# migoox/genome-downsampler

Measured on AMD Instinct MI355X. Metric: Mreads/s selected at target coverage M=100, higher is better.
Workload: dtype u32

## Files before the change

### genome-downsampler_amd/csrc/kernels/pass_major.inc.hip

```cpp
static constexpr int kPmPass = 8192;
__host__ __device__ inline uint32_t pm_stride_of(uint32_t n_ranges) { return (uint32_t)kPmPass + 64u * n_ranges; }
static constexpr int kPmThreads = 512;
static constexpr int kPmWaves = kPmThreads / 64;
static constexpr int kPmPassesPerWg = 4;
static constexpr size_t kPmSortLds = ((size_t)kPmPass + kPmWaves * 256 + 2 * 256 + 16 + 2 * kPmPassesPerWg * 256 + kPmWaves * 3 * 128) * sizeof(uint32_t);
static constexpr uint32_t kPmExcPerWave = 128;

static constexpr uint32_t kPmFlatDigits = 32;
static constexpr uint32_t kPmStageWords = 10240;
static constexpr uint32_t kPmFlatSlots = 8;
static_assert(kPmStageWords >= (uint32_t)kPmPass + kPmFlatDigits * 63u, "a padded pass of 32 slices fits the stage");
static_assert(kPmStageWords <= (uint32_t)kPmPass + kPmWaves * 3u * kPmExcPerWave, "the stage's tail aliases s_exc and nothing else");
static_assert(kPmFlatDigits == 1u << kPmLaneFormBits, "a pass the lane counts rank is a pass the flat write-out takes");

#ifndef QMCP_PM_MIN_WAVES
#define QMCP_PM_MIN_WAVES 4
#endif
__global__ __launch_bounds__(kPmThreads, QMCP_PM_MIN_WAVES) void k_pm_prepare_sort(
    const uint32_t* __restrict__ starts, const uint32_t* __restrict__ ends, uint32_t n,
    const uint64_t* __restrict__ contig_read_off, const uint64_t* __restrict__ contig_pos_off, uint32_t n_contigs,
    const uint32_t* __restrict__ vbase ,
    uint32_t shift, uint32_t stride ,
    uint16_t* __restrict__ keys16, uint16_t* __restrict__ idx16,
    uint32_t* __restrict__ cnt_tab, uint32_t* __restrict__ lst_tab, uint32_t pitch ,
// ... 298 lines not shown
        for (int x = 1; x < kPmWaves; ++x) { mn = min(mn, s_red[0][x]); mx = max(mx, s_red[1][x]); bad |= s_red[2][x]; }
        if (mn < __hip_atomic_load(&stats[0], __ATOMIC_RELAXED, __HIP_MEMORY_SCOPE_AGENT)) atomicMin(&stats[0], mn);
        if (mx > __hip_atomic_load(&stats[1], __ATOMIC_RELAXED, __HIP_MEMORY_SCOPE_AGENT)) atomicMax(&stats[1], mx);
        if (bad) atomicOr(&stats[2], 1u);
    }
}

static constexpr uint32_t kPmDescrY = 8;
static constexpr uint32_t kPmWorkWords = 256u * kPmDescrY * 2u;

struct PmSlot { uint32_t slot0, nv, pass; };
template <bool kVector>
__device__ __forceinline__ PmSlot pm_unpack(uint32_t dsc, bool has, uint32_t stride) {
    PmSlot s;
    s.pass = dsc >> 15;
    s.slot0 = has ? (kVector ? __umul24(s.pass, stride) : s.pass * stride) + (((dsc >> 6) & 511u) << 6) : 0u;
    s.nv = has ? (dsc & 63u) + 1u : 0u;
    return s;
}

__device__ __forceinline__ void pm_row_part(uint32_t pitch, uint32_t& P_beg, uint32_t& P_end) {
    const uint32_t per = (pitch + kPmDescrY - 1u) / kPmDescrY;
    P_beg = min(pitch, blockIdx.y * per);
    P_end = min(pitch, (blockIdx.y + 1u) * per);
}

__global__ __launch_bounds__(256) void k_pm_row_sums(const uint32_t* __restrict__ cnt_tab, const uint32_t* __restrict__ lstw,
                                                     uint32_t pitch, uint32_t* __restrict__ work) {
    __shared__ uint32_t s_red[2][4];
    const uint32_t d = blockIdx.x;
    uint32_t P_beg, P_end;
    pm_row_part(pitch, P_beg, P_end);
    uint32_t pad = 0, tru = 0;
    for (uint32_t P0 = P_beg + threadIdx.x; P0 < P_end; P0 += 4u * 256u) {
        uint32_t c[4], w[4];
#pragma unroll
        for (int u = 0; u < 4; ++u) {
            const uint32_t P = min(P0 + (uint32_t)u * 256u, P_end - 1u);
            c[u] = cnt_tab[(size_t)d * pitch + P];
            w[u] = lstw[(size_t)d * pitch + P];
        }
#pragma unroll
        for (int u = 0; u < 4; ++u)
            if (P0 + (uint32_t)u * 256u < P_end) { pad += c[u]; tru += w[u] >> 16; }
    }
    pad = wave_sum_u32(pad);
    tru = wave_sum_u32(tru);
    if ((threadIdx.x & 63u) == 0u) { s_red[0][threadIdx.x >> 6] = pad; s_red[1][threadIdx.x >> 6] = tru; }
    __syncthreads();
    if (threadIdx.x == 0) {
        uint32_t* const out = work + ((size_t)d * kPmDescrY + blockIdx.y) * 2u;
        out[0] = s_red[0][0] + s_red[0][1] + s_red[0][2] + s_red[0][3];
        out[1] = s_red[1][0] + s_red[1][1] + s_red[1][2] + s_red[1][3];
    }
}

__global__ __launch_bounds__(256) void k_pm_tables(uint32_t* tab, const uint32_t* __restrict__ lstw, uint32_t pitch,
                                                   uint32_t n_groups ,
                                                   uint32_t* __restrict__ desc, const uint32_t* __restrict__ work,
                                                   uint32_t* __restrict__ range_start,
                                                   uint32_t* __restrict__ max_load ,
                                                   uint32_t* __restrict__ clear16 ) {
    __shared__ uint32_t s_red[4], s_red2[4], s_base, s_tile[2][4][4];
    const uint32_t d = blockIdx.x, y = blockIdx.y, tid = threadIdx.x;
    const uint32_t lane = tid & 63u, wv = tid >> 6;
    const bool first = d == 0u && y == 0u;
    uint32_t rp = 0, rt = 0, before = 0;
    {
        const uint4* const src = reinterpret_cast<const uint4*>(work + (size_t)tid * kPmDescrY * 2u);
        uint4 q[kPmDescrY / 2u];
#pragma unroll
        for (uint32_t k = 0; k < kPmDescrY / 2u; ++k) q[k] = src[k];
#pragma unroll
        for (uint32_t k = 0; k < kPmDescrY / 2u; ++k) {
            if (2u * k < y) before += q[k].x;
            if (2u * k + 1u < y) before += q[k].z;
            rp += q[k].x + q[k].z;
            rt += q[k].y + q[k].w;
        }
    }
    {
        const uint32_t inc = wave_incl_scan_add(rp);
        if (lane == 63u) s_red[wv] = inc;
        __syncthreads();
        uint32_t base = 0;
        for (uint32_t x = 0; x < wv; ++x) base += s_red[x];
        if (tid == d) s_base = base + inc - rp + before;
        if (first && tid == 255u) tab[(size_t)256u * pitch] = base + inc;
        __syncthreads();
    }
    if (first) {
        if (clear16 != nullptr && tid < 16u) clear16[tid] = 0u;
        const uint32_t inc = wave_incl_scan_add(rt);
        const uint32_t mx = wave_max_u32(rt), mxp = wave_max_u32(rp);
        if (lane == 63u) s_red[wv] = inc;
        __syncthreads();
        uint32_t base = 0;
        for (uint32_t x = 0; x < wv; ++x) base += s_red[x];
        range_start[tid] = base + inc - rt;
        if (tid == 255u) range_start[256] = base + inc;
        __syncthreads();
        if (lane == 0u) { s_red[wv] = mx; s_red2[wv] = mxp; }
        __syncthreads();
        if (tid == 0) {
            max_load[0] = max(max(s_red[0], s_red[1]), max(s_red[2], s_red[3]));
            max_load[1] = max(max(s_red2[0], s_red2[1]), max(s_red2[2], s_red2[3])) >> 6;
        }
    }
    uint32_t P_beg, P_end;
    pm_row_part(pitch, P_beg, P_end);
    uint32_t carry = s_base;
    uint32_t round = 0;
    for (uint32_t P0 = P_beg; P0 < P_end; P0 += 4u * 256u, round ^= 1u) {
        uint32_t c[4], w[4], inc[4];
#pragma unroll
        for (int u = 0; u < 4; ++u) {
            const uint32_t P = P0 + (uint32_t)u * 256u + tid;
            const bool in = P < P_end;
            const size_t at = (size_t)d * pitch + min(P, P_end - 1u);
            c[u] = tab[at];
            w[u] = lstw[at];
            if (!in) { c[u] = 0u; w[u] = 0u; }
        }
#pragma unroll
        for (int u = 0; u < 4; ++u) {
            inc[u] = wave_incl_scan_add(c[u]);
            if (lane == 63u) s_tile[round][u][wv] = inc[u];
        }
        __syncthreads();
#pragma unroll
        for (int u = 0; u < 4; ++u) {
            uint32_t base = carry;
            for (uint32_t x = 0; x < wv; ++x) base += s_tile[round][u][x];
            carry += s_tile[round][u][0] + s_tile[round][u][1] + s_tile[round][u][2] + s_tile[round][u][3];
            const uint32_t P = P0 + (uint32_t)u * 256u + tid;
            if (P >= P_end) continue;
            const uint32_t t = base + inc[u] - c[u];
            tab[(size_t)d * pitch + P] = t;
            const uint32_t cnt = w[u] >> 16;
            if (cnt == 0u) continue;
            const uint32_t g = t >> 6;
            const uint32_t n_ws = (cnt + 63u) >> 6;
            for (uint32_t j = 0; j < n_ws; ++j)
                if (g + j < n_groups)
                    desc[g + j] = (P << 15) | (((w[u] & 0xFFFFu) + j) << 6) | (min(64u, cnt - 64u * j) - 1u);
        }
    }
}

__device__ __forceinline__ uint32_t pm_grid_pos0(const uint32_t* __restrict__ grid, uint32_t r) { return grid[r]; }
__device__ __forceinline__ uint32_t pm_grid_live(const uint32_t* __restrict__ grid, uint32_t r) { return grid[kPmGridRows + r]; }
__device__ __forceinline__ uint32_t pm_grid_contig(const uint32_t* __restrict__ grid, uint32_t r) { return grid[2u * kPmGridRows + r]; }

#ifndef QMCP_PM_OFFSETS_U
#define QMCP_PM_OFFSETS_U 8
#endif
__global__ __launch_bounds__(1024) void k_pm_offsets(const uint16_t* __restrict__ keys16, const uint32_t* __restrict__ desc,
                                                     const uint32_t* __restrict__ Tp, uint32_t pitch,
                                                     const uint32_t* __restrict__ range_start ,
                                                     const uint32_t* __restrict__ grid,
                                                     uint32_t shift, uint32_t stride, uint32_t ltot, uint32_t* __restrict__ boff,
                                                     uint32_t* __restrict__ empty_positions) {
    extern __shared__ uint32_t s_cnt32[];
#define PADDED(i) ((i) + ((i) >> 5))
    __shared__ uint32_t s_wsum[16], s_esum[16];
    const uint32_t range = blockIdx.x, width = 1u << shift;
    const uint32_t pos0 = pm_grid_pos0(grid, range), live = pm_grid_live(grid, range);
    const uint32_t lo_p = Tp[(size_t)range * pitch], hi_p = Tp[(size_t)(range + 1) * pitch];
    const uint32_t g0 = lo_p >> 6, n_ws = (hi_p - lo_p) >> 6;
    const uint32_t lo = range_start[range];
    for (uint32_t i = threadIdx.x; i < width; i += blockDim.x) s_cnt32[PADDED(i)] = 0;
    __syncthreads();
    const uint32_t lane = threadIdx.x & 63u, nw = blockDim.x >> 6;
    const uint32_t w = (uint32_t)__builtin_amdgcn_readfirstlane((int)(threadIdx.x >> 6));
    const uint32_t sub = lane >> 4, l16 = lane & 15u;
    constexpr int kU = QMCP_PM_OFFSETS_U;
    const uint32_t n_quads = (n_ws + 3u) >> 2;
    uint32_t dsc[kU];
    auto ask_descriptors = [&](uint32_t q0) {
#pragma unroll
        for (int u = 0; u < kU; ++u) dsc[u] = desc[g0 + min(4u * (q0 + (uint32_t)u * nw) + sub, n_ws - 1u)];
    };
    if (n_ws != 0u) ask_descriptors(w);
    for (uint32_t q0 = w; q0 < n_quads; q0 += kU * nw) {
        uint2 v[kU];
        uint32_t nv[kU];
#pragma unroll
        for (int u = 0; u < kU; ++u) {
            const PmSlot at = pm_unpack<true>(dsc[u], 4u * (q0 + (uint32_t)u * nw) + sub < n_ws, stride);
            nv[u] = at.nv;
            v[u] = *reinterpret_cast<const uint2*>(keys16 + at.slot0 + 4u * l16);
        }
        if (q0 + kU * nw < n_quads) ask_descriptors(q0 + kU * nw);
#pragma unroll
        for (int u = 0; u < kU; ++u) {
            const uint32_t e = 4u * l16;
            if (e < nv[u]) atomicAdd(&s_cnt32[PADDED(v[u].x & 0xFFFFu)], 1u);
            if (e + 1 < nv[u]) atomicAdd(&s_cnt32[PADDED(v[u].x >> 16)], 1u);
            if (e + 2 < nv[u]) atomicAdd(&s_cnt32[PADDED(v[u].y & 0xFFFFu)], 1u);
            if (e + 3 < nv[u]) atomicAdd(&s_cnt32[PADDED(v[u].y >> 16)], 1u);
        }
    }
    __syncthreads();
    const uint32_t per = width >= 1024u ? width >> 10 : 1u;
    const uint32_t firstp = threadIdx.x * per;
    uint32_t sum = 0, empties = 0;
    if (firstp < width)
        for (uint32_t qq = 0; qq < per; ++qq) {
            const uint32_t cq = s_cnt32[PADDED(firstp + qq)];
            sum += cq;
            empties += (cq == 0 && firstp + qq < live) ? 1u : 0u;
        }
    const uint32_t inc = wave_incl_scan_add(sum);
    const uint32_t wv = threadIdx.x >> 6;
    if (lane == 63) s_wsum[wv] = inc;
    if (empty_positions != nullptr) {
        empties = wave_sum_u32(empties);
        if (lane == 0) s_esum[wv] = empties;
    }
    __syncthreads();
    if (empty_positions != nullptr && threadIdx.x == 0) {
        uint32_t total = 0;
        for (uint32_t x = 0; x < nw; ++x) total += s_esum[x];
        if (total != 0) atomicAdd(empty_positions, total);
    }
    uint32_t run = lo + inc - sum;
    for (uint32_t x = 0; x < wv; ++x) run += s_wsum[x];
    if (firstp < width)
        for (uint32_t qq = 0; qq < per; ++qq) {
            const uint32_t cq = s_cnt32[PADDED(firstp + qq)];
            s_cnt32[PADDED(firstp + qq)] = run;
            run += cq;
        }
    __syncthreads();
    for (uint32_t i = threadIdx.x; i < live; i += blockDim.x) boff[pos0 + i] = s_cnt32[PADDED(i)];
    if (range == gridDim.x - 1u && threadIdx.x == 0) boff[ltot] = range_start[kPmGridRows];
#undef PADDED
}

struct EvQuota { const uint32_t* sev; const uint32_t* lastns; const uint64_t* poff; uint32_t n_contigs, ell; };

__device__ __forceinline__ uint32_t pm_settle_groups(const uint16_t* __restrict__ keys16, const uint16_t* __restrict__ idx16,
                                                     const uint32_t* __restrict__ desc, uint32_t g0, uint32_t n_ws,
                                                     uint32_t stride, const uint2* amb, uint32_t namb, uint32_t w,
                                                     uint32_t lane, unsigned long long* __restrict__ mask) {
    const uint64_t gt_mask = lane == 63 ? 0ull : ~((2ull << lane) - 1ull);
    uint32_t kept = 0;
    constexpr int kSteps = 16, kE = 2;
    constexpr uint32_t stride_k = 16;
    for (uint32_t k0 = w; k0 < namb; k0 += kE * stride_k) {
        uint32_t key[kE][kSteps], dscv[kE] , p[kE], skip[kE], c_of[kE];
#pragma unroll
        for (int x = 0; x < kE; ++x) {
            const uint32_t k = k0 + (uint32_t)x * stride_k;
            const uint2 ent = k < namb ? amb[k] : make_uint2(0u, 0u);
            c_of[x] = ent.x >> 15;
            p[x] = k < namb ? ent.x & 0x7FFFu : 0xFFFFFFFFu;
            skip[x] = ent.y;
            const uint32_t ws = 16u * c_of[x] + (lane & 15u);
            dscv[x] = ws < n_ws ? desc[g0 + ws] : 0u;
        }
#pragma unroll
        for (int x = 0; x < kE; ++x) {
#pragma unroll
            for (int t = 0; t < kSteps; ++t) {
                const uint32_t dsc = (uint32_t)__builtin_amdgcn_readlane((int)dscv[x], t);
                key[x][t] = keys16[pm_unpack<false>(dsc, 16u * c_of[x] + (uint32_t)t < n_ws, stride).slot0 + lane];
            }
        }
#pragma unroll
        for (int x = 0; x < kE; ++x) {
#pragma unroll
            for (int t = kSteps - 1; t >= 0; --t) {
                const uint32_t dsc = (uint32_t)__builtin_amdgcn_readlane((int)dscv[x], t);
                const PmSlot at = pm_unpack<false>(dsc, 16u * c_of[x] + (uint32_t)t < n_ws, stride);
                const bool member = lane < at.nv && key[x][t] == p[x];
                const uint64_t m = __ballot(member);
                if (m == 0) continue;
                const uint32_t above = (uint32_t)__popcll(m & gt_mask);
                if (member && above >= skip[x]) {
                    const uint32_t v = at.pass * (uint32_t)kPmPass + idx16[at.slot0 + lane];
                    atomicOr(&mask[v >> 6], 1ull << (v & 63u));
                }
                const uint32_t in_step = (uint32_t)__popcll(m);
                kept += in_step > skip[x] ? in_step - skip[x] : 0u;
                skip[x] = skip[x] > in_step ? skip[x] - in_step : 0u;
            }
        }
    }
    return kept;
}

__global__ __launch_bounds__(1024) void k_pm_walk(const uint16_t* __restrict__ keys16, const uint16_t* __restrict__ idx16,
                                                  const uint32_t* __restrict__ desc,
                                                  const uint32_t* __restrict__ Tp, uint32_t pitch,
                                                  const uint32_t* __restrict__ range_start ,
                                                  const uint32_t* __restrict__ grid,
                                                  uint32_t shift, uint32_t stride,
                                                  const uint32_t* __restrict__ boff, const uint32_t* __restrict__ selend,
                                                  EvQuota evq,
                                                  unsigned long long* __restrict__ mask,
                                                  uint2* __restrict__ amb_lists, int lists_by_records,
                                                  unsigned long long* __restrict__ kept_total) {
    extern __shared__ int32_t s_q[];
    __shared__ uint32_t s_namb, s_kept;
    __shared__ uint32_t s_ring[16][128];
    const uint32_t range = blockIdx.x, width = 1u << shift;
    const uint32_t pos0 = pm_grid_pos0(grid, range), live = pm_grid_live(grid, range);
    const uint32_t tid = threadIdx.x, nthreads = blockDim.x;
    const uint32_t lane = tid & 63u;
    const uint32_t w = (uint32_t)__builtin_amdgcn_readfirstlane((int)(tid >> 6));
    const uint32_t lo_p = Tp[(size_t)range * pitch];
    const uint32_t hi_p = Tp[(size_t)(range + 1) * pitch];
    if (lo_p >= hi_p) return;
    const uint32_t g0 = lo_p >> 6, n_ws = (hi_p - lo_p) >> 6;
    const uint32_t n_chunks = (n_ws + 15u) >> 4;
    const uint32_t lo_true = range_start[range];
    uint2* const amb = amb_lists + (lists_by_records ? (size_t)lo_true : (size_t)range * width);
    if (evq.sev != nullptr) {
        const uint32_t c_range = pm_grid_contig(grid, range);
        for (uint32_t i0 = tid; i0 < live; i0 += 8 * nthreads) {
            uint32_t src[8], back[8];
#pragma unroll
            for (int u = 0; u < 8; ++u) {
                const uint32_t p = pos0 + min(i0 + u * nthreads, live - 1);
                uint32_t c_lo = c_range, c_hi = c_range + 1u;
                if (c_range == kPmNoContig) { c_lo = 0; c_hi = evq.n_contigs; }
                while (c_hi - c_lo > 1) {
                    const uint32_t mid = (c_lo + c_hi) >> 1;
                    if ((uint32_t)evq.poff[mid] <= p) c_lo = mid; else c_hi = mid;
                }
                const uint32_t base = (uint32_t)evq.poff[c_lo];
                const uint32_t k = (p - base) / evq.ell;
                src[u] = p;
                back[u] = k - evq.lastns[(size_t)(base / (4u * evq.ell) + c_lo) * 4u + k];
            }
#pragma unroll
            for (int u = 0; u < 8; ++u) src[u] = evq.sev[src[u] - back[u] * evq.ell];
#pragma unroll
            for (int u = 0; u < 8; ++u)
                if (i0 + u * nthreads < live) s_q[i0 + u * nthreads] = (int32_t)src[u];
        }
    } else
    for (uint32_t i0 = tid; i0 < live; i0 += 8 * nthreads) {
        uint32_t a[8], b[8];
#pragma unroll
        for (int u = 0; u < 8; ++u) {
            const uint32_t i = min(i0 + u * nthreads, live - 1);
            a[u] = selend[pos0 + i];
            b[u] = boff[pos0 + i];
        }
#pragma unroll
        for (int u = 0; u < 8; ++u)
            if (i0 + u * nthreads < live) s_q[i0 + u * nthreads] = (int32_t)(a[u] - b[u]);
    }
    if (tid == 0) { s_namb = 0; s_kept = 0; }
    __syncthreads();

#define QMCP_PM_RING "v96", "v97", "v98", "v99", "v100", "v101", "v102", "v103", "v104", "v105", "v106", "v107", "v108", "v109", "v110", "v111", "v112", "v113", "v114", "v115", "v116", "v117", "v118", "v119"
#define QMCP_PM_KEYREG(k) "v" QMCP_PM_STR(QMCP_PM_CAT(QMCP_PM_KEY_, k))
#define QMCP_PM_DSCREG(k) "v" QMCP_PM_STR(QMCP_PM_CAT(QMCP_PM_DSC_, k))
#define QMCP_PM_IDXREG(k) "v" QMCP_PM_STR(QMCP_PM_CAT(QMCP_PM_IDX_, k))
#define QMCP_PM_STR(x) QMCP_PM_STR2(x)
#define QMCP_PM_STR2(x) #x
#define QMCP_PM_CAT(a, b) QMCP_PM_CAT2(a, b)
#define QMCP_PM_CAT2(a, b) a##b
#define QMCP_PM_KEY_0 96
#define QMCP_PM_KEY_1 97
#define QMCP_PM_KEY_2 98
#define QMCP_PM_KEY_3 99
#define QMCP_PM_KEY_4 100
#define QMCP_PM_KEY_5 101
#define QMCP_PM_KEY_6 102
#define QMCP_PM_KEY_7 103
#define QMCP_PM_DSC_0 104
#define QMCP_PM_DSC_1 105
#define QMCP_PM_DSC_2 106
#define QMCP_PM_DSC_3 107
#define QMCP_PM_DSC_4 108
#define QMCP_PM_DSC_5 109
#define QMCP_PM_DSC_6 110
#define QMCP_PM_DSC_7 111
#define QMCP_PM_IDX_0 112
#define QMCP_PM_IDX_1 113
#define QMCP_PM_IDX_2 114
#define QMCP_PM_IDX_3 115
#define QMCP_PM_IDX_4 116
#define QMCP_PM_IDX_5 117
#define QMCP_PM_IDX_6 118
#define QMCP_PM_IDX_7 119
    static_assert(kRankDepth == 8, "the ring registers are named for eight slots");
    struct Slot { uint32_t slot0, nv, read0; bool has; };
    auto desc_offset = [&](uint32_t c) -> uint32_t {
        return (g0 + min(16u * c + w, n_ws - 1u)) * 4u;
    };
    auto slot_of = [&](uint32_t dsc, uint32_t c) -> Slot {
        const bool has = 16u * c + w < n_ws;
        const PmSlot at = pm_unpack<true>(dsc, has, stride);
        Slot s;
        s.slot0 = at.slot0;
        s.nv = at.nv;
        s.read0 = at.pass * (uint32_t)kPmPass;
        s.has = has;
        return s;
    };
    uint32_t kept = 0;
    uint32_t cur = 0, flushed = 0;
    uint32_t* const ring = s_ring[w];
#define QMCP_PM_STEP(K, KF)                                                                                                   \
    {                                                                                                                         \
        const uint32_t c = c0 + (uint32_t)(K);                                                                                \
        uint32_t key, dsc, idx;                                                                                               \
        asm volatile("s_waitcnt vmcnt(19)\n\tv_mov_b32 %0, " QMCP_PM_KEYREG(K) "\n\tv_mov_b32 %1, " QMCP_PM_DSCREG(K)          \
                     "\n\tv_mov_b32 %2, " QMCP_PM_IDXREG(K)                                                                   \
                     : "=v"(key), "=v"(dsc), "=v"(idx) : : QMCP_PM_RING, "memory");                                                      \
        const Slot at = S[K];                                                                                                 \
        const bool valid = lane < at.nv;                                                                                      \
        int32_t old = 0;                                                                                                      \
        if (valid) old = atomicSub(&s_q[key], 1);                                         \
        S[KF] = slot_of(dsc, c + 7u);                                                                                         \
        asm volatile("global_load_ushort " QMCP_PM_KEYREG(KF) ", %0, %1\n\tglobal_load_ushort " QMCP_PM_IDXREG(KF) ", %0, %2"   \
                     "\n\tglobal_load_dword " QMCP_PM_DSCREG(K) ", %3, %4"                                                    \
                     : : "v"((S[KF].slot0 + lane) * 2u), "s"(keys16), "s"(idx16), "v"(desc_offset(c + 15u)), "s"(desc)        \
                     : QMCP_PM_RING, "memory");                                                                               \
        __syncthreads();                                                                                                      \
        int32_t aft = 0;                                                                                                      \
        if (valid) aft = s_q[key];                                                                                            \
        const bool keep = valid && old > 0 && aft >= 0;                                                                       \
        if (valid && old == 1 && aft < 0) {                                                                                   \
            const uint32_t k = atomicAdd(&s_namb, 1u);                                                                        \
            amb[k] = make_uint2((c << 15) | key, (uint32_t)(-aft));                                 \
        }                                                                                                                     \
        __syncthreads();                                               \
        if (at.has) {                                                    \
            const uint64_t kb = __ballot(keep);                                                                               \
            const uint32_t cw = (uint32_t)__popcll(kb);                                                                       \
            if (keep) ring[(cur + __builtin_amdgcn_mbcnt_hi((uint32_t)(kb >> 32), __builtin_amdgcn_mbcnt_lo((uint32_t)kb, 0u))) & 127u] = at.read0 + idx; \
            cur += cw;                                                                                                        \
            if (cur - flushed >= 64u) {                                                                          \
                const uint32_t v = ring[(flushed + lane) & 127u];                                                             \
                atomicOr(&mask[v >> 6], 1ull << (v & 63u));                                                                   \
                flushed += 64u;                                                                                               \
            }                                                                                                                 \
        }                                                                                                                     \
    }
    Slot S[kRankDepth];
    {
        uint32_t d0[kRankDepth - 1];
#pragma unroll
        for (int k = 0; k < kRankDepth - 1; ++k) d0[k] = desc[desc_offset((uint32_t)k) / 4u];
#pragma unroll
        for (int k = 0; k < kRankDepth - 1; ++k) S[k] = slot_of(d0[k], (uint32_t)k);
        S[kRankDepth - 1] = Slot{0u, 0u, 0u, false};
#define QMCP_PM_ASK_KEYS(K) asm volatile("global_load_ushort " QMCP_PM_KEYREG(K) ", %0, %1\n\tglobal_load_ushort " QMCP_PM_IDXREG(K) ", %0, %2" : : "v"((S[K].slot0 + lane) * 2u), "s"(keys16), "s"(idx16) : QMCP_PM_RING, "memory");
#define QMCP_PM_ASK_DSC(K) asm volatile("global_load_dword " QMCP_PM_DSCREG(K) ", %0, %1" : : "v"(desc_offset(7u + (uint32_t)(K))), "s"(desc) : QMCP_PM_RING, "memory");
        QMCP_PM_ASK_KEYS(0) QMCP_PM_ASK_KEYS(1) QMCP_PM_ASK_KEYS(2) QMCP_PM_ASK_KEYS(3) QMCP_PM_ASK_KEYS(4) QMCP_PM_ASK_KEYS(5) QMCP_PM_ASK_KEYS(6)
        QMCP_PM_ASK_DSC(0) QMCP_PM_ASK_DSC(1) QMCP_PM_ASK_DSC(2) QMCP_PM_ASK_DSC(3) QMCP_PM_ASK_DSC(4) QMCP_PM_ASK_DSC(5) QMCP_PM_ASK_DSC(6) QMCP_PM_ASK_DSC(7)
        asm volatile("s_waitcnt vmcnt(0)" : : : QMCP_PM_RING, "memory");
#undef QMCP_PM_ASK_KEYS
#undef QMCP_PM_ASK_DSC
    }
    for (uint32_t c0 = 0; c0 < n_chunks; c0 += kRankDepth) {
        QMCP_PM_STEP(0, 7) QMCP_PM_STEP(1, 0) QMCP_PM_STEP(2, 1) QMCP_PM_STEP(3, 2)
        QMCP_PM_STEP(4, 3) QMCP_PM_STEP(5, 4) QMCP_PM_STEP(6, 5) QMCP_PM_STEP(7, 6)
    }
#undef QMCP_PM_STEP
    asm volatile("s_waitcnt vmcnt(0)" : : : QMCP_PM_RING, "memory");
    if (lane < cur - flushed) {
        const uint32_t v = ring[(flushed + lane) & 127u];
        atomicOr(&mask[v >> 6], 1ull << (v & 63u));
    }
    kept = cur;
    __syncthreads();
    kept += pm_settle_groups(keys16, idx16, desc, g0, n_ws, stride, amb, s_namb, w, lane, mask);
    if (lane == 0 && kept) atomicAdd(&s_kept, kept);
    __syncthreads();
    if (tid == 0 && s_kept) atomicAdd(kept_total, (unsigned long long)s_kept);
}

uint32_t pm_pitch(uint32_t n) { return part_pass_pitch(n); }
uint32_t pm_pass() { return (uint32_t)kPmPass; }
uint32_t pm_stride(uint32_t n_ranges) { return pm_stride_of(n_ranges); }
size_t pm_slots(uint32_t n, uint32_t n_ranges) { return (size_t)pm_pitch(n) * pm_stride(n_ranges); }
uint32_t pm_work_words() { return kPmWorkWords; }
uint32_t pm_exc_slots(uint32_t n) { return pm_pitch(n) * kPmWaves * kPmExcPerWave + kNuOverflow; }
bool pm_rank_scratch_by_records(uint32_t shift, uint32_t n_ranges, uint32_t n) { return (size_t)n < ((size_t)n_ranges << shift); }
size_t pm_rank_scratch_bytes(uint32_t shift, uint32_t n_ranges, uint32_t n) {
    const size_t by_pos = (size_t)n_ranges << shift;
    return (by_pos < (size_t)n ? by_pos : (size_t)n) * sizeof(uint2) + 64;
}
void launch_pm_prepare_sort(hipStream_t st, const uint32_t* starts, const uint32_t* ends, uint32_t n,
                            const uint64_t* d_roff, const uint64_t* d_poff, uint32_t n_contigs, uint32_t shift,
                            uint32_t n_ranges, const uint32_t* d_grid,
                            uint16_t* keys16, uint16_t* idx16, uint32_t* cnt_tab, uint32_t* lst_tab,
                            uint32_t* stats, unsigned long long* zero_mask, uint32_t ell_reg, uint32_t* exc,
                            uint32_t exc_cap, uint32_t* exc_cnt) {
    const uint32_t pitch = pm_pitch(n);
    if (pitch == 0) return;
    (void)hipFuncSetAttribute((const void*)k_pm_prepare_sort, hipFuncAttributeMaxDynamicSharedMemorySize, (int)kPmSortLds);
    hipLaunchKernelGGL(k_pm_prepare_sort, dim3(pitch / kPmPassesPerWg), dim3(kPmThreads), kPmSortLds, st, starts, ends, n,
                       d_roff, d_poff, n_contigs, d_grid + 3u * kPmGridRows, shift, pm_stride(n_ranges), keys16, idx16,
                       cnt_tab, lst_tab, pitch, stats, zero_mask, exc != nullptr ? ell_reg : 0u, exc, exc_cap, exc_cnt);
    if (exc != nullptr && ell_reg != 0u)
        hipLaunchKernelGGL(k_nu_count_groups, dim3(32), dim3(256), 0, st, exc_cnt, pitch * kPmWaves, stats);
}
void launch_pm_row_sums(hipStream_t st, const uint32_t* cnt_tab, const uint32_t* lstw, uint32_t n, uint32_t* work) {
    const uint32_t pitch = pm_pitch(n);
    if (pitch == 0) return;
    hipLaunchKernelGGL(k_pm_row_sums, dim3(256, kPmDescrY), dim3(256), 0, st, cnt_tab, lstw, pitch, work);
}
void launch_pm_tables(hipStream_t st, uint32_t* tab, const uint32_t* lstw, uint32_t n, uint32_t n_ranges,
                      uint32_t* desc, const uint32_t* work, uint32_t* range_start, uint32_t* max_load, uint32_t* clear16) {
    const uint32_t pitch = pm_pitch(n);
    if (pitch == 0) return;
    const uint32_t s64 = pm_stride(n_ranges) / 64u;
    hipLaunchKernelGGL(k_pm_tables, dim3(256, kPmDescrY), dim3(256), 0, st, tab, lstw, pitch, pitch * s64, desc, work,
                       range_start, max_load, clear16);
}
void launch_pm_offsets(hipStream_t st, const uint16_t* keys16, const uint32_t* desc, const uint32_t* Tp, uint32_t n,
                       const uint32_t* range_start, uint32_t shift, uint32_t n_ranges, const uint32_t* d_grid, uint32_t ltot,
                       uint32_t* boff, uint32_t* empty_positions) {
    const size_t width = (size_t)1 << shift;
    const size_t lds = (width + width / 32 + 1) * sizeof(uint32_t);
    (void)hipFuncSetAttribute((const void*)k_pm_offsets, hipFuncAttributeMaxDynamicSharedMemorySize, (int)lds);
    hipLaunchKernelGGL(k_pm_offsets, dim3(n_ranges), dim3(1024), lds, st, keys16, desc, Tp, pm_pitch(n), range_start, d_grid,
                       shift, pm_stride(n_ranges), ltot, boff, empty_positions);
}
void launch_pm_walk(hipStream_t st, const uint16_t* keys16, const uint16_t* idx16, const uint32_t* desc, const uint32_t* Tp,
                    uint32_t n, const uint32_t* range_start, uint32_t shift, uint32_t n_ranges, const uint32_t* d_grid,
                    const uint32_t* boff, const uint32_t* selend, unsigned long long* mask, unsigned long long* kept_total, void* scratch,
                    bool scratch_by_records, const uint32_t* ev_sev, const uint32_t* ev_lastns,
                    const uint64_t* d_poff, uint32_t n_contigs, uint32_t ell) {
    const EvQuota evq{ev_sev, ev_lastns, d_poff, n_contigs, ell};
    const size_t lds = (((size_t)1 << shift) + 1) * sizeof(uint32_t);
    (void)hipFuncSetAttribute((const void*)k_pm_walk, hipFuncAttributeMaxDynamicSharedMemorySize, (int)lds);
    hipLaunchKernelGGL(k_pm_walk, dim3(n_ranges), dim3(1024), lds, st, keys16, idx16, desc, Tp, pm_pitch(n), range_start, d_grid, shift,
                       pm_stride(n_ranges), boff, selend, evq, mask, (uint2*)scratch, scratch_by_records ? 1 : 0,
                       kept_total);
}
```

### genome-downsampler_amd/csrc/qmcp_kernels.hip

```cpp
#include <hip/hip_runtime.h>
#include <stdint.h>

#include <type_traits>

#include "qmcp_kernels.h"
#include "target_table.h"

namespace qmcp {

static constexpr int kWave = 64;
static constexpr uint32_t kInf = 0x40000000u;

#include "kernels/wave_primitives.inc.hip"
#include "kernels/prepare_scan.inc.hip"
#include "kernels/radix_sort.inc.hip"
#include "kernels/ranked_route.inc.hip"
#include "kernels/bucket_offsets.inc.hip"
#include "kernels/sweep_uniform.inc.hip"
#include "kernels/sweep_segments.inc.hip"
#include "kernels/sweep_uniform_pipelines.inc.hip"
#include "kernels/sweep_uniform_events.inc.hip"
#include "kernels/sweep_mixed.inc.hip"
#include "kernels/mark_and_next_rows.inc.hip"
#include "kernels/launchers.inc.hip"
#include "kernels/pm_lane_rank.inc.hip"
#include "kernels/pass_major.inc.hip"
#include "kernels/near_uniform.inc.hip"
#include "kernels/by_contig.inc.hip"
#include "kernels/ladder.inc.hip"
#include "kernels/amplicon_by_contig.inc.hip"
#include "kernels/quality_cells.inc.hip"
#include "kernels/targets.inc.hip"
#include "kernels/depth_report.inc.hip"
#include "kernels/depth_track.inc.hip"
#include "kernels/stratified.inc.hip"
#include "kernels/dedup.inc.hip"
#include "kernels/start_cap.inc.hip"
#include "kernels/profile.inc.hip"
#include "kernels/pairs.inc.hip"
#include "kernels/templates.inc.hip"
#include "kernels/templates_profile.inc.hip"
#include "kernels/fragments.inc.hip"
#include "kernels/ceiling.inc.hip"
#include "kernels/proportional.inc.hip"
#include "kernels/budget.inc.hip"
#include "kernels/mean_depth.inc.hip"
#include "kernels/thresholds.inc.hip"
#include "kernels/replicates.inc.hip"

}
```

Before: 134,300.

## Pipeline pass-major offset counting, settling, and event quotas; add stamp probes

```diff
diff --git a/genome-downsampler_amd/csrc/kernels/pass_major.inc.hip b/genome-downsampler_amd/csrc/kernels/pass_major.inc.hip
--- a/genome-downsampler_amd/csrc/kernels/pass_major.inc.hip
+++ b/genome-downsampler_amd/csrc/kernels/pass_major.inc.hip
@@ -474,8 +474,44 @@
 __device__ __forceinline__ uint32_t pm_grid_live(const uint32_t* __restrict__ grid, uint32_t r) { return grid[kPmGridRows + r]; }
 __device__ __forceinline__ uint32_t pm_grid_contig(const uint32_t* __restrict__ grid, uint32_t r) { return grid[2u * kPmGridRows + r]; }
 
+#ifdef QMCP_PM_STAMP
+__device__ unsigned long long g_pm_stamps[2][kPmGridRows][8];
+__device__ __forceinline__ unsigned long long pm_stamp() {
+    unsigned long long t;
+    asm volatile("s_memtime %0\n\ts_waitcnt lgkmcnt(0)" : "=s"(t) : : "memory");
+    return t;
+}
+__device__ __forceinline__ unsigned long long pm_stamp_after(uint32_t dep) {
+    unsigned long long t;
+    asm volatile("s_memtime %0\n\ts_waitcnt lgkmcnt(0)" : "=s"(t) : "v"(dep) : "memory");
+    return t;
+}
+__device__ __forceinline__ unsigned long long pm_stamp_real() {
+    unsigned long long t;
+    asm volatile("s_memrealtime %0\n\ts_waitcnt lgkmcnt(0)" : "=s"(t) : : "memory");
+    return t;
+}
+#define QMCP_PM_STAMPS unsigned long long pm_t[5] = {0, 0, 0, 0, 0}; const unsigned long long pm_r0 = pm_stamp_real();
+#define QMCP_PM_STAMP_AT(i) pm_t[i] = pm_stamp();
+#define QMCP_PM_STAMP_AFTER(i, dep) pm_t[i] = pm_stamp_after(dep);
+#define QMCP_PM_STAMPS_OUT(kernel)                                                                         \
+    if (threadIdx.x == 0) {                                                                                \
+        unsigned long long* const row = g_pm_stamps[kernel][blockIdx.x];                                   \
+        for (int i = 0; i < 5; ++i) row[i] = pm_t[i];                                                      \
+        row[5] = 1ull; row[6] = pm_r0; row[7] = pm_stamp_real();                                           \
+    }
+#else
+#define QMCP_PM_STAMPS
+#define QMCP_PM_STAMP_AT(i)
+#define QMCP_PM_STAMP_AFTER(i, dep)
+#define QMCP_PM_STAMPS_OUT(kernel)
+#endif
+
+#ifndef QMCP_PM_OFFSETS_REC
+#define QMCP_PM_OFFSETS_REC 8
+#endif
 #ifndef QMCP_PM_OFFSETS_U
-#define QMCP_PM_OFFSETS_U 8
+#define QMCP_PM_OFFSETS_U 4
 #endif
 __global__ __launch_bounds__(1024) void k_pm_offsets(const uint16_t* __restrict__ keys16, const uint32_t* __restrict__ desc,
                                                      const uint32_t* __restrict__ Tp, uint32_t pitch,
@@ -483,47 +519,70 @@
                                                      const uint32_t* __restrict__ grid,
                                                      uint32_t shift, uint32_t stride, uint32_t ltot, uint32_t* __restrict__ boff,
                                                      uint32_t* __restrict__ empty_positions) {
-    extern __shared__ uint32_t s_cnt32[];
+    extern __shared__ __align__(16) uint32_t s_cnt32[];
 #define PADDED(i) ((i) + ((i) >> 5))
     __shared__ uint32_t s_wsum[16], s_esum[16];
     const uint32_t range = blockIdx.x, width = 1u << shift;
+    QMCP_PM_STAMPS
+    QMCP_PM_STAMP_AT(0)
     const uint32_t pos0 = pm_grid_pos0(grid, range), live = pm_grid_live(grid, range);
     const uint32_t lo_p = Tp[(size_t)range * pitch], hi_p = Tp[(size_t)(range + 1) * pitch];
     const uint32_t g0 = lo_p >> 6, n_ws = (hi_p - lo_p) >> 6;
     const uint32_t lo = range_start[range];
-    for (uint32_t i = threadIdx.x; i < width; i += blockDim.x) s_cnt32[PADDED(i)] = 0;
-    __syncthreads();
     const uint32_t lane = threadIdx.x & 63u, nw = blockDim.x >> 6;
     const uint32_t w = (uint32_t)__builtin_amdgcn_readfirstlane((int)(threadIdx.x >> 6));
-    const uint32_t sub = lane >> 4, l16 = lane & 15u;
     constexpr int kU = QMCP_PM_OFFSETS_U;
-    const uint32_t n_quads = (n_ws + 3u) >> 2;
+    constexpr uint32_t kRec = QMCP_PM_OFFSETS_REC;
+    static_assert(kRec == 4 || kRec == 8, "a lane loads 8 or 16 bytes");
+    const uint32_t sub = lane / (64u / kRec), l_in = lane % (64u / kRec);
+    const uint32_t n_groups = (n_ws + kRec - 1u) / kRec, step = (uint32_t)kU * nw;
     uint32_t dsc[kU];
     auto ask_descriptors = [&](uint32_t q0) {
 #pragma unroll
-        for (int u = 0; u < kU; ++u) dsc[u] = desc[g0 + min(4u * (q0 + (uint32_t)u * nw) + sub, n_ws - 1u)];
+        for (int u = 0; u < kU; ++u) dsc[u] = desc[g0 + min(kRec * (q0 + (uint32_t)u * nw) + sub, n_ws - 1u)];
+    };
+    uint32_t v[kU][kRec / 2], nv[kU];
+    auto ask_round = [&](uint32_t q0) {
+#pragma unroll
+        for (int u = 0; u < kU; ++u) {
+            const PmSlot at = pm_unpack<true>(dsc[u], kRec * (q0 + (uint32_t)u * nw) + sub < n_ws, stride);
+            nv[u] = at.nv;
+            const uint16_t* const src = keys16 + at.slot0 + kRec * l_in;
+            if constexpr (kRec == 4) {
+                const uint2 x = *reinterpret_cast<const uint2*>(src);
+                v[u][0] = x.x; v[u][1] = x.y;
+            } else {
+                const uint4 x = *reinterpret_cast<const uint4*>(src);
+                v[u][0] = x.x; v[u][1] = x.y; v[u][2] = x.z; v[u][3] = x.w;
+            }
+        }
+        ask_descriptors(q0 + step);
     };
     if (n_ws != 0u) ask_descriptors(w);
-    for (uint32_t q0 = w; q0 < n_quads; q0 += kU * nw) {
-        uint2 v[kU];
-        uint32_t nv[kU];
+    const uint32_t n_words = width + (width >> 5), n_vec = n_words >> 2, half = (n_vec + 1u) >> 1;
+    uint4* const cnt4 = reinterpret_cast<uint4*>(s_cnt32);
+    for (uint32_t i = threadIdx.x; i < half; i += blockDim.x) cnt4[i] = make_uint4(0u, 0u, 0u, 0u);
+    if (w < n_groups) ask_round(w);
+    for (uint32_t i = half + threadIdx.x; i < n_vec; i += blockDim.x) cnt4[i] = make_uint4(0u, 0u, 0u, 0u);
+    for (uint32_t i = 4u * n_vec + threadIdx.x; i < n_words; i += blockDim.x) s_cnt32[i] = 0u;
+    __syncthreads();
+    for (uint32_t q0 = w; q0 < n_groups; q0 += step) {
+#ifdef QMCP_PM_STAMP
+        if (q0 == w) QMCP_PM_STAMP_AFTER(1, v[kU - 1][kRec / 2 - 1])
+#endif
 #pragma unroll
         for (int u = 0; u < kU; ++u) {
-            const PmSlot at = pm_unpack<true>(dsc[u], 4u * (q0 + (uint32_t)u * nw) + sub < n_ws, stride);
-            nv[u] = at.nv;
-            v[u] = *reinterpret_cast<const uint2*>(keys16 + at.slot0 + 4u * l16);
-        }
-        if (q0 + kU * nw < n_quads) ask_descriptors(q0 + kU * nw);
-#pragma unroll
-        for (int u = 0; u < kU; ++u) {
-            const uint32_t e = 4u * l16;
-            if (e < nv[u]) atomicAdd(&s_cnt32[PADDED(v[u].x & 0xFFFFu)], 1u);
-            if (e + 1 < nv[u]) atomicAdd(&s_cnt32[PADDED(v[u].x >> 16)], 1u);
-            if (e + 2 < nv[u]) atomicAdd(&s_cnt32[PADDED(v[u].y & 0xFFFFu)], 1u);
-            if (e + 3 < nv[u]) atomicAdd(&s_cnt32[PADDED(v[u].y >> 16)], 1u);
-        }
+            const uint32_t e = kRec * l_in;
+#pragma unroll
+            for (uint32_t x = 0; x < kRec / 2; ++x) {
+                if (e + 2u * x < nv[u]) atomicAdd(&s_cnt32[PADDED(v[u][x] & 0xFFFFu)], 1u);
+                if (e + 2u * x + 1u < nv[u]) atomicAdd(&s_cnt32[PADDED(v[u][x] >> 16)], 1u);
+            }
+        }
+        if (q0 + step < n_groups) ask_round(q0 + step);
     }
     __syncthreads();
+    QMCP_PM_STAMP_AT(2)
     const uint32_t per = width >= 1024u ? width >> 10 : 1u;
     const uint32_t firstp = threadIdx.x * per;
     uint32_t sum = 0, empties = 0;
@@ -555,12 +614,49 @@
             run += cq;
         }
     __syncthreads();
+    QMCP_PM_STAMP_AT(3)
     for (uint32_t i = threadIdx.x; i < live; i += blockDim.x) boff[pos0 + i] = s_cnt32[PADDED(i)];
     if (range == gridDim.x - 1u && threadIdx.x == 0) boff[ltot] = range_start[kPmGridRows];
+    QMCP_PM_STAMP_AT(4)
+    QMCP_PM_STAMPS_OUT(0)
 #undef PADDED
 }
 
-struct EvQuota { const uint32_t* sev; const uint32_t* lastns; const uint64_t* poff; uint32_t n_contigs, ell; };
+struct EvQuota { const uint32_t* sev; const uint32_t* lastns; const uint64_t* poff; uint32_t n_contigs, ell; PmDiv div; };
+
+template <int kQ, bool kOne>
+__device__ __forceinline__ void pm_event_quotas(const EvQuota& evq, uint32_t c_range, uint32_t pos0, uint32_t live, uint32_t tid,
+                                                uint32_t nthreads, int32_t* s_q) {
+    uint32_t base_u = 0, row_u = 0;
+    if (kOne) {
+        base_u = (uint32_t)evq.poff[c_range];
+        row_u = (pm_div(base_u, evq.div) >> 2) + c_range;
+    }
+    for (uint32_t i0 = tid; i0 < live; i0 += kQ * nthreads) {
+        uint32_t val[kQ];
+#pragma unroll
+        for (int u = 0; u < kQ; ++u) {
+            const uint32_t p = pos0 + min(i0 + u * nthreads, live - 1);
+            uint32_t base = base_u, row = row_u;
+            if (!kOne) {
+                uint32_t c_lo = 0, c_hi = evq.n_contigs;
+                while (c_hi - c_lo > 1) {
+                    const uint32_t mid = (c_lo + c_hi) >> 1;
+                    if ((uint32_t)evq.poff[mid] <= p) c_lo = mid; else c_hi = mid;
+                }
+                base = (uint32_t)evq.poff[c_lo];
+                row = (pm_div(base, evq.div) >> 2) + c_lo;
+            }
+            const uint32_t k = pm_div(p - base, evq.div);
+            val[u] = k - evq.lastns[(size_t)row * 4u + k];
+        }
+#pragma unroll
+        for (int u = 0; u < kQ; ++u) val[u] = evq.sev[pos0 + min(i0 + u * nthreads, live - 1) - val[u] * evq.ell];
+#pragma unroll
+        for (int u = 0; u < kQ; ++u)
+            if (i0 + u * nthreads < live) s_q[i0 + u * nthreads] = (int32_t)val[u];
+    }
+}
 
 __device__ __forceinline__ uint32_t pm_settle_groups(const uint16_t* __restrict__ keys16, const uint16_t* __restrict__ idx16,
                                                      const uint32_t* __restrict__ desc, uint32_t g0, uint32_t n_ws,
@@ -568,47 +664,97 @@
                                                      uint32_t lane, unsigned long long* __restrict__ mask) {
     const uint64_t gt_mask = lane == 63 ? 0ull : ~((2ull << lane) - 1ull);
     uint32_t kept = 0;
-    constexpr int kSteps = 16, kE = 2;
+    constexpr int kSteps = 16;
     constexpr uint32_t stride_k = 16;
-    for (uint32_t k0 = w; k0 < namb; k0 += kE * stride_k) {
-        uint32_t key[kE][kSteps], dscv[kE] , p[kE], skip[kE], c_of[kE];
-#pragma unroll
-        for (int x = 0; x < kE; ++x) {
-            const uint32_t k = k0 + (uint32_t)x * stride_k;
-            const uint2 ent = k < namb ? amb[k] : make_uint2(0u, 0u);
-            c_of[x] = ent.x >> 15;
-            p[x] = k < namb ? ent.x & 0x7FFFu : 0xFFFFFFFFu;
-            skip[x] = ent.y;
-            const uint32_t ws = 16u * c_of[x] + (lane & 15u);
-            dscv[x] = ws < n_ws ? desc[g0 + ws] : 0u;
-        }
-#pragma unroll
-        for (int x = 0; x < kE; ++x) {
+    struct Group {
+        uint32_t key[kSteps];
+        uint32_t dscv;
+        uint32_t c, p, skip;
+    };
+    struct Kept {
+        uint32_t idx[kSteps];
+        uint32_t marked;
+        uint32_t dscv;
+    };
+    const uint32_t mine = namb > w ? (namb - w + stride_k - 1u) / stride_k : 0u;
+    for (uint32_t j0 = 0; j0 < mine; j0 += 64u) {
+        const uint32_t nj = min(64u, mine - j0);
+        const uint32_t k_lane = w + stride_k * (j0 + lane);
+        const uint2 ent = k_lane < namb ? amb[k_lane] : make_uint2(0u, 0u);
+        uint32_t dsc_next;
+        auto ask_descriptors = [&](uint32_t j) {
+            const uint32_t c = (uint32_t)__builtin_amdgcn_readlane((int)ent.x, (int)min(j, nj - 1u)) >> 15;
+            const uint32_t ws = 16u * c + (lane & 15u);
+            dsc_next = desc[g0 + min(ws, n_ws - 1u)];
+        };
+        auto ask_positions = [&](Group& G, uint32_t j) {
+            const int jj = (int)min(j, nj - 1u);
+            const uint32_t e = (uint32_t)__builtin_amdgcn_readlane((int)ent.x, jj);
+            G.c = e >> 15;
+            G.p = e & 0x7FFFu;
+            G.skip = (uint32_t)__builtin_amdgcn_readlane((int)ent.y, jj);
+            G.dscv = dsc_next;
 #pragma unroll
             for (int t = 0; t < kSteps; ++t) {
-                const uint32_t dsc = (uint32_t)__builtin_amdgcn_readlane((int)dscv[x], t);
-                key[x][t] = keys16[pm_unpack<false>(dsc, 16u * c_of[x] + (uint32_t)t < n_ws, stride).slot0 + lane];
-            }
-        }
-#pragma unroll
-        for (int x = 0; x < kE; ++x) {
+                const uint32_t dsc = (uint32_t)__builtin_amdgcn_readlane((int)G.dscv, t);
+                G.key[t] = keys16[pm_unpack<false>(dsc, 16u * G.c + (uint32_t)t < n_ws, stride).slot0 + lane];
+            }
+        };
+        auto walk = [&](const Group& G, Kept& K) {
+            uint32_t skip = G.skip;
+            K.marked = 0u;
+            K.dscv = G.dscv;
 #pragma unroll
             for (int t = kSteps - 1; t >= 0; --t) {
-                const uint32_t dsc = (uint32_t)__builtin_amdgcn_readlane((int)dscv[x], t);
-                const PmSlot at = pm_unpack<false>(dsc, 16u * c_of[x] + (uint32_t)t < n_ws, stride);
-                const bool member = lane < at.nv && key[x][t] == p[x];
+                const uint32_t dsc = (uint32_t)__builtin_amdgcn_readlane((int)G.dscv, t);
+                const PmSlot at = pm_unpack<false>(dsc, 16u * G.c + (uint32_t)t < n_ws, stride);
+                const bool member = lane < at.nv && G.key[t] == G.p;
                 const uint64_t m = __ballot(member);
+                K.idx[t] = 0u;
                 if (m == 0) continue;
                 const uint32_t above = (uint32_t)__popcll(m & gt_mask);
-                if (member && above >= skip[x]) {
-                    const uint32_t v = at.pass * (uint32_t)kPmPass + idx16[at.slot0 + lane];
-                    atomicOr(&mask[v >> 6], 1ull << (v & 63u));
+                if (member && above >= skip) {
+                    K.idx[t] = idx16[at.slot0 + lane];
+                    K.marked |= 1u << t;
                 }
                 const uint32_t in_step = (uint32_t)__popcll(m);
-                kept += in_step > skip[x] ? in_step - skip[x] : 0u;
-                skip[x] = skip[x] > in_step ? skip[x] - in_step : 0u;
-            }
-        }
+                kept += in_step > skip ? in_step - skip : 0u;
+                skip = skip > in_step ? skip - in_step : 0u;
+            }
+        };
+        auto mark = [&](Kept& K) {
+            if (__ballot(K.marked != 0u) != 0) {
+#pragma unroll
+                for (int t = 0; t < kSteps; ++t)
+                    if ((K.marked >> t) & 1u) {
+                        const uint32_t v = ((uint32_t)__builtin_amdgcn_readlane((int)K.dscv, t) >> 15) * (uint32_t)kPmPass + K.idx[t];
+                        atomicOr(&mask[v >> 6], 1ull << (v & 63u));
+                    }
+            }
+            K.marked = 0u;
+        };
+        Group A, B;
+        Kept KA, KB;
+        KA.marked = KB.marked = 0u;
+        KA.dscv = KB.dscv = 0u;
+#pragma unroll
+        for (int t = 0; t < kSteps; ++t) KA.idx[t] = KB.idx[t] = 0u;
+        ask_descriptors(0u);
+        ask_positions(A, 0u);
+        ask_descriptors(1u);
+        for (uint32_t j = 0; j < nj; j += 2u) {
+            ask_positions(B, j + 1u);
+            ask_descriptors(j + 2u);
+            walk(A, KA);
+            mark(KB);
+            if (j + 1u >= nj) break;
+            ask_positions(A, j + 2u);
+            ask_descriptors(j + 3u);
+            walk(B, KB);
+            mark(KA);
+        }
+        mark(KA);
+        mark(KB);
     }
     return kept;
 }
@@ -632,6 +778,8 @@
     const uint32_t tid = threadIdx.x, nthreads = blockDim.x;
     const uint32_t lane = tid & 63u;
     const uint32_t w = (uint32_t)__builtin_amdgcn_readfirstlane((int)(tid >> 6));
+    QMCP_PM_STAMPS
+    QMCP_PM_STAMP_AT(0)
     const uint32_t lo_p = Tp[(size_t)range * pitch];
     const uint32_t hi_p = Tp[(size_t)(range + 1) * pitch];
     if (lo_p >= hi_p) return;
@@ -639,30 +787,13 @@
     const uint32_t n_chunks = (n_ws + 15u) >> 4;
     const uint32_t lo_true = range_start[range];
     uint2* const amb = amb_lists + (lists_by_records ? (size_t)lo_true : (size_t)range * width);
+    uint32_t d0[kRankDepth - 1];
+#pragma unroll
+    for (int k = 0; k < kRankDepth - 1; ++k) d0[k] = desc[g0 + min(16u * (uint32_t)k + w, n_ws - 1u)];
     if (evq.sev != nullptr) {
         const uint32_t c_range = pm_grid_contig(grid, range);
-        for (uint32_t i0 = tid; i0 < live; i0 += 8 * nthreads) {
-            uint32_t src[8], back[8];
-#pragma unroll
-            for (int u = 0; u < 8; ++u) {
-                const uint32_t p = pos0 + min(i0 + u * nthreads, live - 1);
-                uint32_t c_lo = c_range, c_hi = c_range + 1u;
-                if (c_range == kPmNoContig) { c_lo = 0; c_hi = evq.n_contigs; }
-                while (c_hi - c_lo > 1) {
-                    const uint32_t mid = (c_lo + c_hi) >> 1;
-                    if ((uint32_t)evq.poff[mid] <= p) c_lo = mid; else c_hi = mid;
-                }
-                const uint32_t base = (uint32_t)evq.poff[c_lo];
-                const uint32_t k = (p - base) / evq.ell;
-                src[u] = p;
-                back[u] = k - evq.lastns[(size_t)(base / (4u * evq.ell) + c_lo) * 4u + k];
-            }
-#pragma unroll
-            for (int u = 0; u < 8; ++u) src[u] = evq.sev[src[u] - back[u] * evq.ell];
-#pragma unroll
-            for (int u = 0; u < 8; ++u)
-                if (i0 + u * nthreads < live) s_q[i0 + u * nthreads] = (int32_t)src[u];
-        }
+        if (c_range != kPmNoContig) pm_event_quotas<16, true>(evq, c_range, pos0, live, tid, nthreads, s_q);
+        else pm_event_quotas<8, false>(evq, c_range, pos0, live, tid, nthreads, s_q);
     } else
     for (uint32_t i0 = tid; i0 < live; i0 += 8 * nthreads) {
         uint32_t a[8], b[8];
@@ -768,9 +899,6 @@
     }
     Slot S[kRankDepth];
     {
-        uint32_t d0[kRankDepth - 1];
-#pragma unroll
-        for (int k = 0; k < kRankDepth - 1; ++k) d0[k] = desc[desc_offset((uint32_t)k) / 4u];
 #pragma unroll
         for (int k = 0; k < kRankDepth - 1; ++k) S[k] = slot_of(d0[k], (uint32_t)k);
         S[kRankDepth - 1] = Slot{0u, 0u, 0u, false};
@@ -782,12 +910,14 @@
 #undef QMCP_PM_ASK_KEYS
 #undef QMCP_PM_ASK_DSC
     }
+    QMCP_PM_STAMP_AT(1)
     for (uint32_t c0 = 0; c0 < n_chunks; c0 += kRankDepth) {
         QMCP_PM_STEP(0, 7) QMCP_PM_STEP(1, 0) QMCP_PM_STEP(2, 1) QMCP_PM_STEP(3, 2)
         QMCP_PM_STEP(4, 3) QMCP_PM_STEP(5, 4) QMCP_PM_STEP(6, 5) QMCP_PM_STEP(7, 6)
     }
 #undef QMCP_PM_STEP
     asm volatile("s_waitcnt vmcnt(0)" : : : QMCP_PM_RING, "memory");
+    QMCP_PM_STAMP_AT(2)
     if (lane < cur - flushed) {
         const uint32_t v = ring[(flushed + lane) & 127u];
         atomicOr(&mask[v >> 6], 1ull << (v & 63u));
@@ -797,9 +927,16 @@
     kept += pm_settle_groups(keys16, idx16, desc, g0, n_ws, stride, amb, s_namb, w, lane, mask);
     if (lane == 0 && kept) atomicAdd(&s_kept, kept);
     __syncthreads();
+    QMCP_PM_STAMP_AT(3)
+    QMCP_PM_STAMPS_OUT(1)
     if (tid == 0 && s_kept) atomicAdd(kept_total, (unsigned long long)s_kept);
 }
 
+#ifdef QMCP_PM_STAMP
+extern "C" int qmcp_lab_pm_stamps(unsigned long long* out) {
+    return (int)hipMemcpyFromSymbol(out, HIP_SYMBOL(g_pm_stamps), sizeof(g_pm_stamps));
+}
+#endif
 uint32_t pm_pitch(uint32_t n) { return part_pass_pitch(n); }
 uint32_t pm_pass() { return (uint32_t)kPmPass; }
 uint32_t pm_stride(uint32_t n_ranges) { return pm_stride_of(n_ranges); }
@@ -853,7 +990,7 @@
                     const uint32_t* boff, const uint32_t* selend, unsigned long long* mask, unsigned long long* kept_total, void* scratch,
                     bool scratch_by_records, const uint32_t* ev_sev, const uint32_t* ev_lastns,
                     const uint64_t* d_poff, uint32_t n_contigs, uint32_t ell) {
-    const EvQuota evq{ev_sev, ev_lastns, d_poff, n_contigs, ell};
+    const EvQuota evq{ev_sev, ev_lastns, d_poff, n_contigs, ell, pm_div_make(ell)};
     const size_t lds = (((size_t)1 << shift) + 1) * sizeof(uint32_t);
     (void)hipFuncSetAttribute((const void*)k_pm_walk, hipFuncAttributeMaxDynamicSharedMemorySize, (int)lds);
     hipLaunchKernelGGL(k_pm_walk, dim3(n_ranges), dim3(1024), lds, st, keys16, idx16, desc, Tp, pm_pitch(n), range_start, d_grid, shift,
diff --git a/genome-downsampler_amd/csrc/pm_div.h b/genome-downsampler_amd/csrc/pm_div.h
--- /dev/null
+++ b/genome-downsampler_amd/csrc/pm_div.h
@@ -0,0 +1,34 @@
+#pragma once
+#include <cstdint>
+
+#if defined(__HIPCC__) || defined(__CUDACC__)
+#define QMCP_PM_DIV_HD __host__ __device__
+#else
+#define QMCP_PM_DIV_HD
+#endif
+
+namespace qmcp {
+
+static constexpr uint32_t kPmDivMaxDivisor = 512u;
+static constexpr uint32_t kPmDivMaxDividend = 0x7FFFFFFFu;
+
+struct PmDiv { uint32_t mul, shift; };
+
+QMCP_PM_DIV_HD inline PmDiv pm_div_make(uint32_t d) {
+    if (d == 0u) d = 1u;
+    uint32_t s = 0;
+    while ((1u << s) < d) ++s;
+    const uint64_t two = 1ull << (32u + s);
+    const uint64_t M = (two + d - 1u) / d;
+    return PmDiv{(uint32_t)(M - (1ull << 32)), s};
+}
+
+QMCP_PM_DIV_HD inline uint32_t pm_div(uint32_t n, PmDiv k) {
+#if defined(__HIP_DEVICE_COMPILE__)
+    return (__umulhi(n, k.mul) + n) >> k.shift;
+#else
+    return ((uint32_t)(((uint64_t)n * k.mul) >> 32) + n) >> k.shift;
+#endif
+}
+
+}
diff --git a/genome-downsampler_amd/csrc/qmcp_kernels.hip b/genome-downsampler_amd/csrc/qmcp_kernels.hip
--- a/genome-downsampler_amd/csrc/qmcp_kernels.hip
+++ b/genome-downsampler_amd/csrc/qmcp_kernels.hip
@@ -5,6 +5,7 @@
 
 #include "qmcp_kernels.h"
 #include "target_table.h"
+#include "pm_div.h"
 
 namespace qmcp {
 
diff --git a/lab/pm_range_stamps.py b/lab/pm_range_stamps.py
--- /dev/null
+++ b/lab/pm_range_stamps.py
@@ -0,0 +1,42 @@
+import ctypes, hashlib, importlib, os, sys
+import numpy as np
+R = os.path.dirname(os.path.dirname(os.path.abspath(__file__))); sys.path.insert(0, R)
+pkg = importlib.import_module('genome-downsampler_amd')
+import torch
+ss, ee = [], []
+for c in range(8):
+    a, b = pkg.reads_gen(0, 6_250_000, 1_000_000, seed=12345 + c); ss.append(a); ee.append(b)
+S = np.concatenate(ss); E = np.concatenate(ee)
+offs = np.arange(9, dtype=np.uint64) * 12_500_000
+lengths = np.full(8, 1_000_000, np.uint32)
+sv = pkg.Solver(0)
+dS = torch.from_numpy(S.view(np.int32)).cuda(); dE = torch.from_numpy(E.view(np.int32)).cuda()
+dM = torch.zeros((S.size + 63) // 64, dtype=torch.int64, device="cuda")
+lib = ctypes.CDLL(pkg.HIP_LIB_PATH)
+if not hasattr(lib, "qmcp_lab_pm_stamps"):
+    sys.exit("this library has no stamps: build it with -DQMCP_PM_STAMP and name it in QMCP_HIP_LIB")
+PHASES = {0: [("entry -> first count", 0, 1), ("counting loop", 1, 2), ("scan", 2, 3), ("boff store issued", 3, 4), ("whole", 0, 4)],
+          1: [("entry -> first draw", 0, 1), ("walk loop", 1, 2), ("tail (settling)", 2, 3), ("whole", 0, 3)]}
+rows = {0: {}, 1: {}}
+for it in range(8):
+    sv.solve_device(dS.data_ptr(), dE.data_ptr(), S.size, lengths, 100, dM.data_ptr(), contig_read_offsets=offs)
+    torch.cuda.synchronize()
+    if it < 3:
+        continue
+    st = np.zeros(2 * 256 * 8, np.uint64)
+    assert lib.qmcp_lab_pm_stamps(st.ctypes.data_as(ctypes.POINTER(ctypes.c_ulonglong))) == 0
+    st = st.reshape(2, 256, 8).astype(np.float64)
+    for k in (0, 1):
+        t = st[k][st[k][:, 5] == 1]
+        us_per_tick = (t[:, 7] - t[:, 6]) / 100.0 / (t[:, 4 if k == 0 else 3] - t[:, 0])
+        for name, a, b in PHASES[k]:
+            rows[k].setdefault(name, []).append(np.percentile((t[:, b] - t[:, a]) * np.median(us_per_tick), [50, 10, 90]))
+        rows[k].setdefault("shader clock, MHz", []).append(np.full(3, 1.0 / np.median(us_per_tick)))
+        rows[k].setdefault("workgroups", []).append(np.full(3, float(len(t))))
+m = dM.cpu().numpy()
+print("kept %d  mask sha1 %s" % (sv.last_stats.as_dict()['n_kept'], hashlib.sha1(m.tobytes()).hexdigest()[:12]))
+for k, kern in ((0, "k_pm_offsets"), (1, "k_pm_walk")):
+    print(kern + "  (median over ranges: median / 10th / 90th percentile, us; mean of 5 solves)")
+    for name, v in rows[k].items():
+        a = np.mean(np.array(v), axis=0)
+        print("   %-24s %9.2f %9.2f %9.2f" % (name, a[0], a[1], a[2]))
```

Result: faster. 136,500, median of 6 (+1.6%).
